# boqian-li/GarmentDreamer

Measured on AMD Instinct MI355X. Metric: SDS iters/sec (rasterize+UNet+bwd), 100k Gaussians ×8 views @512², 1/2/4/8 GPU, higher is better.
Workload: dtype bf16

## Files before the change

garmentdreamer_amd/csrc/nn_conv3x3.hip:

```cpp
#include <hip/hip_runtime.h>
#include <stdlib.h>
#include <stdint.h>
#include <stdio.h>

#include <mutex>
#include <vector>

#include "../../include/gd_nn.h"
#include "nn_device.h"
#include "nn_host.h"

#ifndef GD_CONV_ABLATE
#define GD_CONV_ABLATE 0
#endif

namespace {

using namespace gdnn;

#ifndef GD_PATCH_EPI
#define GD_PATCH_EPI 0
#endif
typedef __attribute__((ext_vector_type(4))) float f32x4;

// ... 241 lines not shown

__device__ __forceinline__ float silu_fast(float z) { return z * __builtin_amdgcn_rcpf(1.0f + __expf(-z)); }

__device__ __forceinline__ float row16_sum(float v)
{
    v += __builtin_bit_cast(float, __builtin_amdgcn_update_dpp(0, __builtin_bit_cast(int, v), 0xB1, 0xf, 0xf, false));
    v += __builtin_bit_cast(float, __builtin_amdgcn_update_dpp(0, __builtin_bit_cast(int, v), 0x4E, 0xf, 0xf, false));
    v += __builtin_bit_cast(float, __builtin_amdgcn_update_dpp(0, __builtin_bit_cast(int, v), 0x141, 0xf, 0xf, false));
    v += __builtin_bit_cast(float, __builtin_amdgcn_update_dpp(0, __builtin_bit_cast(int, v), 0x140, 0xf, 0xf, false));
    return v;
}

__device__ __forceinline__ void stat_accumulate(float2& st, uint2 o)
{
    const float r0 = __uint_as_float(o.x << 16), r1 = __uint_as_float(o.x & 0xffff0000u);
    const float r2 = __uint_as_float(o.y << 16), r3 = __uint_as_float(o.y & 0xffff0000u);
    st.x += (r0 + r1) + (r2 + r3);
    st.y += fmaf(r0, r0, fmaf(r1, r1, fmaf(r2, r2, r3 * r3)));
}

__device__ __forceinline__ void patch_col(int fn, int& rr, int& fx)
{
    if (fn < 4) { rr = 0; fx = fn; }
    else if (fn < 12) { rr = 1; fx = fn - 4; }
    else if (fn < 16) { rr = 0; fx = fn - 8; }
    else if (fn < 20) { rr = 1; fx = fn - 8; }
    else if (fn < 28) { rr = 0; fx = fn - 12; }
    else { rr = 1; fx = fn - 16; }
}

constexpr int kTrRow = 80;
constexpr int kTrWave = 64 * kTrRow;

template <int BN, int WN, int FA, int FB>
__device__ __forceinline__ void patch_epilogue(f32x16 (&acc)[FA][FB], char* tr, int nimg, int tyi, int txi, int n0, int wc,
                                               int wp, int lane, int H, int W, int Cout, const uint16_t* __restrict__ bias,
                                               int bias_img_stride, const uint16_t* __restrict__ residual,
                                               uint16_t* __restrict__ out, float* __restrict__ stat_part, int tpi,
                                               int tiles_x)
{
    const int fk = lane >> 5, fn = lane & 31;
    int rr, fx;
    patch_col(fn, rr, fx);
    bool ok[FB];
    size_t opix[FB];
#pragma unroll
    for (int b = 0; b < FB; b++) {
        const int oy = tyi * 16 + 4 * wp + 2 * b + rr, ox = txi * 16 + fx;
        ok[b] = oy < H && ox < W;
        opix[b] = ((size_t)nimg * H + oy) * W + ox;
    }
    const uint16_t* bias_n = bias ? bias + (size_t)nimg * bias_img_stride : nullptr;
    const int stat_rows = tpi * 8;
    const int stat_row = (tyi * tiles_x + txi) * 8 + wp * 2 + ((lane >> 4) & 1);
    const bool wide = GD_PATCH_EPI != 2 && tr != nullptr && (Cout & 7) == 0;
#pragma unroll
    for (int a = 0; a < FA; a++) {
#pragma unroll
        for (int q = 0; q < 4; q++) {
            const int co = n0 + wc * (BN / WN) + a * 32 + 8 * q + 4 * fk;
            const bool cok = co < Cout;
            float bv[4] = {0.f, 0.f, 0.f, 0.f};
            if (bias_n && cok) {
                const uint2 bb = *(const uint2*)(bias_n + co);
                bv[0] = bf2f((uint16_t)(bb.x & 0xffff)); bv[1] = bf2f((uint16_t)(bb.x >> 16));
                bv[2] = bf2f((uint16_t)(bb.y & 0xffff)); bv[3] = bf2f((uint16_t)(bb.y >> 16));
// ... 13 lines not shown
                uint2 o;
                o.x = pack_bf16(v[0], v[1]);
                o.y = pack_bf16(v[2], v[3]);
                if (wide) *(uint2*)(tr + (b * 32 + fn) * kTrRow + 16 * q + 8 * fk) = o;
                else if (GD_PATCH_EPI != 1 || H < 0) *(uint2*)(out + opix[b] * Cout + co) = o;
                if (stat_part) stat_accumulate(st, o);
            }
            if (stat_part) {
                const float sx = row16_sum(st.x), sy = row16_sum(st.y);
                if ((lane & 15) == 0 && cok)
                    *(float2*)(stat_part + (((size_t)nimg * (Cout >> 2) + (co >> 2)) * stat_rows + stat_row) * 2) =
                        make_float2(sx, sy);
            }
        }
        if (wide) {
            __builtin_amdgcn_wave_barrier();
#pragma unroll
            for (int i = 0; i < FB * 2; i++) {
                const int pr = (lane >> 2) + 16 * i, ch = lane & 3;
                int rr2, fx2;
                patch_col(pr & 31, rr2, fx2);
                const int oy = tyi * 16 + 4 * wp + 2 * (pr >> 5) + rr2, ox = txi * 16 + fx2;
                const int co8 = n0 + wc * (BN / WN) + a * 32 + 8 * ch;
                if (oy < H && ox < W && co8 < Cout) {
                    const uint4 v = *(const uint4*)(tr + pr * kTrRow + ch * 16);
                    if (GD_PATCH_EPI != 1 || H < 0) *(uint4*)(out + (((size_t)nimg * H + oy) * W + ox) * Cout + co8) = v;
                }
            }
            __builtin_amdgcn_wave_barrier();
        }
    }
}

template <int BN, int WN, int WM, bool GN>
__global__ __launch_bounds__(64 * WN * WM) void conv3x3_gn_patch_kernel(
    const uint16_t* __restrict__ in, const uint16_t* __restrict__ wt, const uint16_t* __restrict__ bias,
    int bias_img_stride, const uint16_t* __restrict__ residual, uint16_t* __restrict__ out, int Nimg, int H, int W,
    int Cin, int Cout, const float* __restrict__ mean_rstd, const uint16_t* __restrict__ gamma,
    const uint16_t* __restrict__ beta, int G, int apply_silu, int tiles_n, int tiles_x, int tiles_y, int nwg,
    float* __restrict__ stat_part)
{
    constexpr int BM = 256;
    constexpr int THREADS = 64 * WN * WM;
    constexpr int NB = BN * 8 / THREADS;
    constexpr int NA = (kPatchPix * 8 + THREADS - 1) / THREADS;
    constexpr int FA = BN / WN / 32, FB = BM / WM / 32;
    static_assert(FB == 2 && THREADS % 8 == 0, "wave pixel block = 4 patch rows x 16");
    constexpr int kAStage = (kPatchPix + 4) * BK * 2;
    constexpr int kBStage = BN * BK * 2;
    extern __shared__ __attribute__((aligned(16))) char smem[];
    char* sA = smem;
    char* sB = smem + 2 * kAStage;

    const int tid = threadIdx.x, lane = tid & 63;
    const int wave = __builtin_amdgcn_readfirstlane(tid >> 6);
    int bid = blockIdx.x;
    if ((nwg & 7) == 0) bid = (bid & 7) * (nwg >> 3) + (bid >> 3);
    const int tn = bid % tiles_n, tm = bid / tiles_n;
    const int tpi = tiles_x * tiles_y;
    const int nimg = tm / tpi, trem = tm - nimg * tpi;
    const int tyi = trem / tiles_x, txi = trem - tyi * tiles_x;
    const int y0 = tyi * 16 - 1, x0 = txi * 16 - 1;
    const int n0 = tn * BN;

    const uint32_t row_bytes = (uint32_t)Cin * 2u;
    const __amdgpu_buffer_rsrc_t rs_in = buffer_rsrc(in, (uint32_t)Nimg * (uint32_t)(H * W) * row_bytes);
    const __amdgpu_buffer_rsrc_t rs_w = buffer_rsrc(wt, (uint32_t)Cout * 9u * row_bytes);
// ... 72 lines not shown
#pragma unroll
    for (int a = 0; a < FA; a++)
#pragma unroll
        for (int b = 0; b < FB; b++)
#pragma unroll
            for (int k = 0; k < 16; k++) acc[a][b][k] = 0.f;

    const int wc = wave % WN, wp = wave / WN;
    const int fk = lane >> 5, fn = lane & 31;
    int rr, fx;
    if (fn < 4) { rr = 0; fx = fn; }
    else if (fn < 12) { rr = 1; fx = fn - 4; }
    else if (fn < 16) { rr = 0; fx = fn - 8; }
    else if (fn < 20) { rr = 1; fx = fn - 8; }
    else if (fn < 28) { rr = 0; fx = fn - 12; }
    else { rr = 1; fx = fn - 16; }
    uint32_t w_rd[FA];
    int p_base[FB];
#pragma unroll
    for (int a = 0; a < FA; a++) w_rd[a] = (uint32_t)swz(wc * (BN / WN) + a * 32 + fn, fk);
#pragma unroll
    for (int b = 0; b < FB; b++) p_base[b] = (4 * wp + 2 * b + rr) * kPatch + fx;

    const int kc = Cin / BK;
    const int nsteps = 9 * kc;
    auto issueA = [&](int buf, int c) {
        char* dst = sA + buf * kAStage;
#pragma unroll
        for (int i = 0; i < NA; i++) {
            if (i == NA - 1 && wave * 64 + THREADS * i >= kPatchPix * 8) continue;
            bload_lds16(rs_in, a_goff[i], (uint32_t)c * (BK * 2), dst + (wave * 64 + THREADS * i) * 16);
        }
    };
    if (GN) {
        if (mean_rstd) gn_table_fill(tab_off, tid, THREADS, Cin, G, nimg, mean_rstd, gamma, beta);
        loadA(0);
        issueB(0, 0, 0);
        if (mean_rstd) gn_table_sync();
        storeA(0, 0);
    } else {
        issueA(0, 0);
        issueB(0, 0, 0);
    }
    int s = 0;
    for (int c = 0; c < kc; c++) {
        const char* pa = sA + (c & 1) * kAStage;
        for (int tap = 0; tap < 9; tap++, s++) {
            const int bufB = s & 1;
            if (GN) asm volatile("s_waitcnt vmcnt(0) lgkmcnt(0)" ::: "memory");
            else asm volatile("s_waitcnt vmcnt(0)" ::: "memory");
            __syncthreads();
            if (s + 1 < nsteps) issueB(bufB ^ 1, tap == 8 ? 0 : tap + 1, tap == 8 ? c + 1 : c);
            if (c + 1 < kc) {
                if (GN) {
                    if (tap == 0) loadA(c + 1);
                    else if (tap == 1) storeA((c + 1) & 1, c + 1);
                } else if (tap == 0) {
                    issueA((c + 1) & 1, c + 1);
                }
            }
            const char* pb = sB + bufB * kBStage;
            const int tapoff = (tap / 3) * kPatch + (tap % 3);
            uint32_t p_rd[FB], p_sw[FB];
#pragma unroll
            for (int b = 0; b < FB; b++) {
                const int p = p_base[b] + tapoff;
                p_rd[b] = (uint32_t)p * 128u;
                p_sw[b] = (uint32_t)((p >> 1) & 7);
            }
#pragma unroll
            for (int kk = 0; kk < 4; kk++) {
                bf16x8_t wf[FA], pf[FB];
#pragma unroll
                for (int a = 0; a < FA; a++) wf[a] = *(const bf16x8_t*)(pb + (w_rd[a] ^ (uint32_t)(kk << 5)));
#pragma unroll
                for (int b = 0; b < FB; b++)
                    pf[b] = *(const bf16x8_t*)(pa + p_rd[b] + ((((uint32_t)(2 * kk + fk)) ^ p_sw[b]) << 4));
#pragma unroll
                for (int a = 0; a < FA; a++)
#pragma unroll
                    for (int b = 0; b < FB; b++)
                        acc[a][b] = __builtin_amdgcn_mfma_f32_32x32x16_bf16(wf[a], pf[b], acc[a][b], 0, 0, 0);
            }
        }
    }

    if (GD_PATCH_EPI != 2) __syncthreads();
    patch_epilogue<BN, WN, FA, FB>(acc, sA + ((kc - 1) & 1) * kAStage + wave * kTrWave, nimg, tyi, txi, n0, wc, wp, lane, H, W,
                                   Cout, bias, bias_img_stride, residual, out, stat_part, tpi, tiles_x);
}

template <int BN, int WN, int WM, bool GN>
__global__ __launch_bounds__(64 * WN * WM) void conv3x3_patch_stream_kernel(
    const uint16_t* __restrict__ in, const uint16_t* __restrict__ wt, const uint16_t* __restrict__ bias,
    int bias_img_stride, const uint16_t* __restrict__ residual, uint16_t* __restrict__ out, int Nimg, int H, int W,
    int Cin, int Cout, const float* __restrict__ mean_rstd, const uint16_t* __restrict__ gamma,
    const uint16_t* __restrict__ beta, int G, int apply_silu, int tiles_n, int tiles_x, int tiles_y, int nwg,
    float* __restrict__ stat_part)
{
    constexpr int BM = 256;
    constexpr int THREADS = 64 * WN * WM;
    constexpr int NB = BN * 8 / THREADS;
    constexpr int NA = (kPatchPix * 8 + THREADS - 1) / THREADS;
    constexpr int FA = BN / WN / 32, FB = BM / WM / 32;
    static_assert(FB == 2 && THREADS % 8 == 0, "wave pixel block = 4 patch rows x 16");
    constexpr int kAStage = (kPatchPix + 4) * BK * 2;
    constexpr int kBStage = BN * BK * 2;
    extern __shared__ __attribute__((aligned(16))) char smem[];
    char* sA = smem;
    char* sB = smem + 2 * kAStage;

    const int tid = threadIdx.x, lane = tid & 63;
    const int wave = __builtin_amdgcn_readfirstlane(tid >> 6);
    const int tpi = tiles_x * tiles_y;
    const bool remap = (nwg & 7) == 0 && (GN || (gridDim.x & 7) == 0);
    struct Tile { int nimg, tyi, txi, n0; };
    auto decode = [&](int vb) {
        int bid = vb;
        if (remap) bid = (vb & 7) * (nwg >> 3) + (vb >> 3);
        const int tn = bid % tiles_n, tm = bid / tiles_n;
// ... 764 lines not shown
        hipLaunchKernelGGL(kern, dim3(nmax, 1, ncls), dim3(64 * WN_ * WM_), lds, s, (const uint16_t*)x,            \
                           (const uint16_t*)bias, bias_img_stride, (const uint16_t*)residual, (uint16_t*)y, N, gs, \
                           Cin, Cout, tiles_n);                                                                    \
    } while (0)
    if (variant == 2) GD_LAUNCH_M(256, 256, 2, 4);
    else if (variant == 1) GD_LAUNCH_M(128, 256, 2, 4);
    else GD_LAUNCH_M(128, 128, 2, 2);
#undef GD_LAUNCH_M
    prof.close(flops, bytes);
    const int r = launch_status();
    return r < 0 ? r : 1;
}

static int launch_patch(void* stream, const void* x, const float* mean_rstd, const void* gamma, const void* beta,
                        int groups, int apply_silu, const void* weight, const void* bias, int bias_img_stride,
                        const void* residual, void* y, int N, int H, int W, int Cin, int Cout,
                        float* stat_part = nullptr)
{
    if (!x || !weight || !y) return fail(GD_NN_ERR_INVALID_ARG, "null pointer");
    if (N <= 0 || H <= 0 || W <= 0 || Cin % BK || Cout % 4 || Cin <= 0 || Cout <= 0)
        return fail(GD_NN_ERR_INVALID_ARG, "conv3x3_gn: need Cin % 64 == 0 and Cout % 4 == 0");
    if (mean_rstd && (!gamma || !beta || groups <= 0 || Cin % groups))
        return fail(GD_NN_ERR_INVALID_ARG, "conv3x3_gn: GroupNorm needs gamma, beta and Cin % groups == 0");
    if ((double)N * H * W * Cin * 2.0 >= 2147483648.0 || (double)Cout * 9.0 * Cin * 2.0 >= 2147483648.0)
        return fail(GD_NN_ERR_INVALID_ARG, "conv3x3_gn: activation / weight tensor must be < 2 GiB (32-bit buffer offsets)");
    const TiledArgs a = {stream, x, mean_rstd, gamma, beta, groups, apply_silu, weight, bias, bias_img_stride, residual, y,
                         N, H, W, Cin, Cout, stat_part};
    int bn = (Cout % 256 == 0) ? 256 : 128;
    if (g_force_variant == 1 || g_force_variant == 0) bn = 128;
    if (g_force_variant == 2) bn = 256;
    const bool persistent = conv_env().patch_persistent != 0;
    constexpr auto lds = [](int slab) { return 2 * (kPatchPix + 4) * BK * 2 + 2 * slab * BK * 2; };
    if (mean_rstd && bn == 256 && !gn_table_fits(lds(256), Cin)) bn = 128;
    if (bn == 256)
        return mean_rstd ? launch_tiled<conv3x3_gn_patch_kernel<256, 2, 4, true>>(a, lds(256), 16, 256, false)
                         : launch_tiled<conv3x3_patch_stream_kernel<256, 2, 4, false>>(a, lds(256), 16, 256, persistent);
    return mean_rstd ? launch_tiled<conv3x3_gn_patch_kernel<128, 2, 4, true>>(a, lds(128), 16, 128, false)
                     : launch_tiled<conv3x3_patch_stream_kernel<128, 2, 4, false>>(a, lds(128), 16, 128, persistent);
}


static bool prefer_patch(int N, int H, int W, int Cout)
{
    if (g_force_variant >= 0 || g_force_split >= 0) return g_force_variant == 3;
    if (Cout < 64 || H < 16 || W < 16) return false;
    const int bn = Cout % 256 == 0 ? 256 : 128;
    const int64_t wgs = (int64_t)N * g_route_scale * ((H + 15) / 16) * ((W + 15) / 16) * ((Cout + bn - 1) / bn);
    return wgs >= 256;
}

size_t gd_nn_conv3x3_ws_bytes(int N, int H, int W, int Cin, int Cout)
{
    if (N <= 0 || H <= 0 || W <= 0 || Cout <= 0) return 0;
    if (prefer_patch(N, H, W, Cout)) return 0;
    const int64_t M = (int64_t)N * H * W;
    const int split = choose_split(M, Cout, 9, Cin);
    return split > 1 ? split_ws_bytes(split, M, Cout) : 0;
}

int gd_nn_conv_force_split(int s)
{
    g_force_split = s;
    return GD_NN_OK;
}

int gd_nn_conv_set_route_scale(int k)
{
    if (k < 1) return fail(GD_NN_ERR_INVALID_ARG, "conv route scale must be >= 1");
    g_route_scale = k;
    return GD_NN_OK;
}
// ... 60 lines not shown
    return (size_t)((Cout + 127) / 128) * 3 * (size_t)(Cin / kWinoCK) * (size_t)kWinoWStage;
}

int gd_nn_conv3x3_wino_weights(void* stream, const void* weight, void* u, int Cout, int Cin)
{
    if (!weight || !u || Cout <= 0 || Cin <= 0) return fail(GD_NN_ERR_INVALID_ARG, "wino_weights: bad argument");
    if (Cin % kWinoCK) return fail(GD_NN_ERR_INVALID_ARG, "wino_weights: Cin % 32 != 0");
    const size_t total = gd_nn_conv3x3_wino_weights_bytes(Cout, Cin) / 16;
    const int grid = (int)((total + 255) / 256 < 4096 ? (total + 255) / 256 : 4096);
    hipLaunchKernelGGL(conv3x3_wino_weights_kernel, dim3(grid), dim3(256), 0, (hipStream_t)stream, (const uint16_t*)weight,
                       (uint16_t*)u, Cout, Cin);
    return launch_status();
}

int gd_nn_conv3x3_wino_supported(int N, int H, int W, int Cin, int Cout)
{
    if (N <= 0 || H < 16 || W < 16 || Cin <= 0 || Cout < 64) return 0;
    if (Cin % kWinoCK || Cout % 8) return 0;
    if ((double)N * H * W * Cin * 2.0 >= 2147483648.0 || (double)gd_nn_conv3x3_wino_weights_bytes(Cout, Cin) >= 2147483648.0) return 0;
    return 1;
}

static int launch_wino(void* stream, const void* x, const float* mean_rstd, const void* gamma, const void* beta, int groups,
                       int apply_silu, const void* u, const void* bias, int bias_img_stride, const void* residual, void* y,
                       int N, int H, int W, int Cin, int Cout, float* stat_part)
{
    if (!x || !u || !y) return fail(GD_NN_ERR_INVALID_ARG, "null pointer");
    if (!gd_nn_conv3x3_wino_supported(N, H, W, Cin, Cout))
        return fail(GD_NN_ERR_INVALID_ARG, "conv3x3_wino: need Cin % 32 == 0, Cout % 8 == 0, Cout >= 64, H, W >= 16, tensors < 2 GiB");
    if (mean_rstd && (!gamma || !beta || groups <= 0 || Cin % groups))
        return fail(GD_NN_ERR_INVALID_ARG, "conv3x3_wino: GroupNorm needs gamma, beta and Cin % groups == 0");
    const TiledArgs a = {stream, x, mean_rstd, gamma, beta, groups, apply_silu, u, bias, bias_img_stride, residual, y,
                         N, H, W, Cin, Cout, stat_part};
    return mean_rstd ? launch_tiled<conv3x3_wino_kernel<true>>(a, kWinoLds, 16, 128, false)
                     : launch_tiled<conv3x3_wino_kernel<false>>(a, kWinoLds, 16, 128, false);
}

int gd_nn_conv3x3_wino_forward(void* stream, const void* x, const void* u, const void* bias, int bias_img_stride,
                               const void* residual, void* y, int N, int H, int W, int Cin, int Cout, float* stat_part)
{
    return launch_wino(stream, x, nullptr, nullptr, nullptr, 0, 0, u, bias, bias_img_stride, residual, y, N, H, W, Cin,
                       Cout, stat_part);
}

int gd_nn_conv3x3_wino_gn_forward(void* stream, const void* x, const float* mean_rstd, const void* gamma, const void* beta,
                                  int groups, int apply_silu, const void* u, const void* bias, int bias_img_stride,
                                  const void* residual, void* y, int N, int H, int W, int Cin, int Cout, float* stat_part)
{
    if (!mean_rstd) return fail(GD_NN_ERR_INVALID_ARG, "conv3x3_wino_gn: mean_rstd is NULL");
    return launch_wino(stream, x, mean_rstd, gamma, beta, groups, apply_silu, u, bias, bias_img_stride, residual, y, N, H, W,
                       Cin, Cout, stat_part);
}

size_t gd_nn_conv3x3_wide_weights_bytes(int Cout, int Cin)
{
    if (Cout <= 0 || Cin <= 0 || Cin % kWideCK) return 0;
    return (size_t)((Cout + 127) / 128) * 3 * (size_t)(Cin / kWideCK) * (size_t)kWideWStage;
}

int gd_nn_conv3x3_wide_weights(void* stream, const void* weight, void* u, int Cout, int Cin)
{
    if (!weight || !u || Cout <= 0 || Cin <= 0 || Cin % kWideCK) return fail(GD_NN_ERR_INVALID_ARG, "wide_weights: bad argument");
    const size_t total = gd_nn_conv3x3_wide_weights_bytes(Cout, Cin) / 16;
    const int grid = (int)((total + 255) / 256 < 4096 ? (total + 255) / 256 : 4096);
    hipLaunchKernelGGL(conv3x3_wide_weights_kernel, dim3(grid), dim3(256), 0, (hipStream_t)stream, (const uint16_t*)weight,
                       (uint16_t*)u, Cout, Cin);
    return launch_status();
}

#ifdef GD_NN_EXPERIMENTAL_STREAM
#include "nn_conv_stream_api.h"
#endif

int gd_nn_conv3x3_wide_supported(int N, int H, int W, int Cin, int Cout)
{
    if (N <= 0 || H < 16 || W < 16 || Cin <= 0 || Cout < 64) return 0;
    if (Cin % kWideCK || Cout % 8) return 0;
    if ((double)N * H * W * Cin * 2.0 >= 2147483648.0 || (double)gd_nn_conv3x3_wide_weights_bytes(Cout, Cin) >= 2147483648.0) return 0;
    return 1;
}

static int launch_wide(void* stream, const void* x, const float* mean_rstd, const void* gamma, const void* beta, int groups,
                       int apply_silu, const void* u, const void* bias, int bias_img_stride, const void* residual, void* y,
                       int N, int H, int W, int Cin, int Cout, float* stat_part)
{
    if (!x || !u || !y) return fail(GD_NN_ERR_INVALID_ARG, "null pointer");
    if (!gd_nn_conv3x3_wide_supported(N, H, W, Cin, Cout))
        return fail(GD_NN_ERR_INVALID_ARG, "conv3x3_wide: need Cin % 32 == 0, Cout % 8 == 0, Cout >= 64, H, W >= 16, tensors < 2 GiB");
    if (mean_rstd && (!gamma || !beta || groups <= 0 || Cin % groups))
        return fail(GD_NN_ERR_INVALID_ARG, "conv3x3_wide: GroupNorm needs gamma, beta and Cin % groups == 0");
    const TiledArgs a = {stream, x, mean_rstd, gamma, beta, groups, apply_silu, u, bias, bias_img_stride, residual, y,
                         N, H, W, Cin, Cout, stat_part};
    return mean_rstd ? launch_tiled<conv3x3_wide_kernel<true>>(a, kWideLds, 32, 128, false)
                     : launch_tiled<conv3x3_wide_kernel<false>>(a, kWideLds, 32, 128, false);
}

int gd_nn_conv3x3_wide_forward(void* stream, const void* x, const void* u, const void* bias, int bias_img_stride,
                               const void* residual, void* y, int N, int H, int W, int Cin, int Cout, float* stat_part)
{
    return launch_wide(stream, x, nullptr, nullptr, nullptr, 0, 0, u, bias, bias_img_stride, residual, y, N, H, W, Cin,
                       Cout, stat_part);
}

int gd_nn_conv3x3_wide_gn_forward(void* stream, const void* x, const float* mean_rstd, const void* gamma, const void* beta,
                                  int groups, int apply_silu, const void* u, const void* bias, int bias_img_stride,
                                  const void* residual, void* y, int N, int H, int W, int Cin, int Cout, float* stat_part)
{
    if (!mean_rstd) return fail(GD_NN_ERR_INVALID_ARG, "conv3x3_wide_gn: mean_rstd is NULL");
    return launch_wide(stream, x, mean_rstd, gamma, beta, groups, apply_silu, u, bias, bias_img_stride, residual, y, N, H, W,
                       Cin, Cout, stat_part);
}

#ifdef GD_NN_EXPERIMENTAL_REGW
#include "nn_conv_regw_api.h"
#endif

static int first_mfma_grid(int N, int H, int W)
{
    const int64_t tiles = (int64_t)N * H * ((W + 31) / 32);
    int64_t grid = (tiles + 3) / 4;
    const int64_t cap = 512;
    if (grid > cap) grid = cap;
    return (int)(grid < 1 ? 1 : grid);
}

size_t gd_nn_conv3x3_first_stat_rows(int N, int H, int W, int Cin, int Cout)
{
// ... 291 lines not shown
```

garmentdreamer_amd/csrc/nn_conv_wide.h:

```cpp
#pragma once
#include "nn_device.h"

constexpr int kWideCK = 32;
constexpr int kWidePW = 34, kWidePix = 18 * kWidePW;
constexpr int kWidePStage = 2560 * 16;
constexpr int kWideWStage = 3 * 128 * kWideCK * 2;
constexpr int kWideLds = 2 * kWidePStage + 2 * kWideWStage;

__global__ __launch_bounds__(256) void conv3x3_wide_weights_kernel(const uint16_t* __restrict__ w, uint16_t* __restrict__ u,
                                                                   int Cout, int Cin)
{
    const int kc = Cin / kWideCK;
    const int tiles_n = (Cout + 127) / 128;
    const size_t total = (size_t)tiles_n * 3 * kc * 1536;
    for (size_t i = (size_t)blockIdx.x * blockDim.x + threadIdx.x; i < total; i += (size_t)gridDim.x * blockDim.x) {
        const int q = (int)(i % 1536);
        const size_t sl = i / 1536;
        const int c = (int)(sl % kc);
        const int ky = (int)((sl / kc) % 3);
        const int tn = (int)(sl / kc / 3);
        const int pc = q & 3, row = (q >> 2) & 127, kx = q >> 9;
        const int co = tn * 128 + row;
        const int ci0 = c * kWideCK + ((pc ^ ((row >> 2) & 3)) << 3);
        uint4 v = make_uint4(0u, 0u, 0u, 0u);
        if (co < Cout) v = *(const uint4*)(w + (((size_t)co * 3 + ky) * 3 + kx) * Cin + ci0);
        *(uint4*)(u + i * 8) = v;
    }
}

template <bool GN>
__global__ __launch_bounds__(512) void conv3x3_wide_kernel(
    const uint16_t* __restrict__ in, const uint16_t* __restrict__ uw, const uint16_t* __restrict__ bias,
    int bias_img_stride, const uint16_t* __restrict__ residual, uint16_t* __restrict__ out, int Nimg, int H, int W,
    int Cin, int Cout, const float* __restrict__ mean_rstd, const uint16_t* __restrict__ gamma,
    const uint16_t* __restrict__ beta, int G, int apply_silu, int tiles_n, int tiles_x, int tiles_y, int nwg,
    float* __restrict__ stat_part)
{
    constexpr int THREADS = 512;
    typedef __attribute__((ext_vector_type(4))) uint32_t u32x4;
    extern __shared__ __attribute__((aligned(16))) char smem[];
    char* sP = smem;
    char* sW = smem + 2 * kWidePStage;

    const int tid = threadIdx.x, lane = tid & 63;
    const int wave = __builtin_amdgcn_readfirstlane(tid >> 6);
    int bid = blockIdx.x;
    if ((nwg & 7) == 0) bid = (bid & 7) * (nwg >> 3) + (bid >> 3);
    const int tn = bid % tiles_n, tm = bid / tiles_n;
    const int tpi = tiles_x * tiles_y;
    const int nimg = tm / tpi, trem = tm - nimg * tpi;
    const int tyi = trem / tiles_x, txi = trem - tyi * tiles_x;
    const int y0 = tyi * 16 - 1, x0 = txi * 32 - 1;
    const int n0 = tn * 128;

    const uint32_t row_bytes = (uint32_t)Cin * 2u;
    const __amdgpu_buffer_rsrc_t rs_in = buffer_rsrc(in, (uint32_t)Nimg * (uint32_t)(H * W) * row_bytes);
    const int kc = Cin / kWideCK;
    const __amdgpu_buffer_rsrc_t rs_w = buffer_rsrc(uw, (uint32_t)tiles_n * 3u * (uint32_t)kc * (uint32_t)kWideWStage);

    uint32_t p_goff[5];
    uint32_t p_keep = 0;
#pragma unroll
    for (int i = 0; i < 5; i++) {
        const int q = tid + THREADS * i;
        const int pix = q >> 2;
        const int py = (pix * 1928) >> 16, px = pix - py * kWidePW;
        const int gy = y0 + py, gx = x0 + px;
        const bool inimg = (pix < kWidePix) & ((unsigned)gy < (unsigned)H) & ((unsigned)gx < (unsigned)W);
        const int oct = GN ? (q & 3) : (q & 3) ^ ((pix >> 2) & 3);
        p_goff[i] = inimg ? (uint32_t)((nimg * H + gy) * W + gx) * row_bytes + (uint32_t)oct * 16u : kOOB;
        if (inimg) p_keep |= 1u << i;
    }
    auto issueP = [&](int buf, int c) {
        char* dst = sP + buf * kWidePStage;
#pragma unroll
        for (int i = 0; i < 5; i++) {
            if (i == 4 && wave == 7) continue;
            bload_lds16(rs_in, p_goff[i], (uint32_t)c * (kWideCK * 2), dst + (wave * 64 + THREADS * i) * 16);
        }
    };
    u32x4 p_reg[3];
    auto loadP = [&](int c, int i0, int i1) {
#pragma unroll
        for (int i = i0; i < i1; i++) {
            if (i == 4 && wave == 7) continue;
            p_reg[i - i0] = __builtin_bit_cast(u32x4, __builtin_amdgcn_raw_buffer_load_b128(rs_in, (int)p_goff[i],
                                                                                         (int)(c * (kWideCK * 2)), 0));
        }
    };
    const uint32_t sP_off = (uint32_t)(uintptr_t)sP;
    const uint32_t tab_off = (uint32_t)(uintptr_t)(smem + kWideLds);
    auto storeP = [&](int buf, int c, int i0, int i1) {
        float sc[8], sh[8];
        gn_table_read(tab_off, c * (kWideCK / 8) + (tid & 3), sc, sh);
#pragma unroll
        for (int i = i0; i < i1; i++) {
            if (i == 4 && wave == 7) continue;
            const int q = tid + THREADS * i, pix = q >> 2;
            const bool keep = (p_keep >> i) & 1u;
            u32x4 v;
#pragma unroll
            for (int k = 0; k < 4; k++) {
                float lo = __uint_as_float(p_reg[i - i0][k] << 16), hi = __uint_as_float(p_reg[i - i0][k] & 0xffff0000u);
                lo = lo * sc[2 * k] + sh[2 * k];
                hi = hi * sc[2 * k + 1] + sh[2 * k + 1];
                if (apply_silu) { lo = silu_fast(lo); hi = silu_fast(hi); }
                v[k] = keep ? pack_bf16(lo, hi) : 0u;
            }
            asm volatile("ds_write_b128 %0, %1" ::"v"(sP_off + (uint32_t)(buf * kWidePStage) + (uint32_t)pix * 64u +
                                                       (uint32_t)(((q & 3) ^ ((pix >> 2) & 3)) << 4)), "v"(v) : "memory");
        }
    };
    const uint32_t w_voff = (uint32_t)tid * 16u;
    auto issueW = [&](int buf, int ky, int c) {
        char* dst = sW + buf * kWideWStage;
        const uint32_t soff = (uint32_t)((tn * 3 + ky) * kc + c) * (uint32_t)kWideWStage;
#pragma unroll
        for (int i = 0; i < 3; i++)
            bload_lds16(rs_w, w_voff + (uint32_t)(THREADS * 16 * i), soff, dst + (wave * 64 + THREADS * i) * 16);
    };

    const int wc = wave & 1, wr = wave >> 1;
    const int fk = lane >> 5, fn = lane & 31;
    int rr, fx;
    patch_col(fn, rr, fx);
    f32x16 acc[2][4];
#pragma unroll
    for (int a = 0; a < 2; a++)
#pragma unroll
        for (int b = 0; b < 4; b++)
#pragma unroll
            for (int k = 0; k < 16; k++) acc[a][b][k] = 0.f;
    int p_base[4];
#pragma unroll
    for (int b = 0; b < 4; b++) p_base[b] = (4 * wr + 2 * (b & 1) + rr) * kWidePW + 16 * (b >> 1) + fx;
    uint32_t a_rd[2];
#pragma unroll
    for (int a = 0; a < 2; a++) a_rd[a] = (uint32_t)((wc * 64 + a * 32 + fn) * 64);
    const uint32_t a_key = (uint32_t)((fn >> 2) & 3);

    const int nsteps = 3 * kc;
    if (GN) {
        gn_table_fill(tab_off, tid, THREADS, Cin, G, nimg, mean_rstd, gamma, beta);
        loadP(0, 0, 3);
        gn_table_sync();
        storeP(0, 0, 0, 3); loadP(0, 3, 5); storeP(0, 0, 3, 5);
    } else {
        issueP(0, 0);
    }
    issueW(0, 0, 0);
    int s = 0;
    for (int c = 0; c < kc; c++) {
        const char* pa = sP + (c & 1) * kWidePStage;
        for (int ky = 0; ky < 3; ky++, s++) {
            const int bufW = s & 1;
            asm volatile("s_waitcnt vmcnt(0) lgkmcnt(0)" ::: "memory");
            __syncthreads();
            if (s + 1 < nsteps) issueW(bufW ^ 1, ky == 2 ? 0 : ky + 1, ky == 2 ? c + 1 : c);
            if (c + 1 < kc) {
                if (GN) {
                    if (ky == 0) loadP(c + 1, 0, 3);
                    else if (ky == 1) { storeP((c + 1) & 1, c + 1, 0, 3); loadP(c + 1, 3, 5); }
                    else storeP((c + 1) & 1, c + 1, 3, 5);
                } else if (ky == 0) {
                    issueP((c + 1) & 1, c + 1);
                }
            }
            const char* pw = sW + bufW * kWideWStage;
#pragma unroll 1
            for (int kx = 0; kx < 3; kx++) {
                uint32_t p_rd[4], p_sw[4];
#pragma unroll
                for (int b = 0; b < 4; b++) {
                    const int p = p_base[b] + ky * kWidePW + kx;
                    p_rd[b] = (uint32_t)p * 64u;
                    p_sw[b] = (uint32_t)((p >> 2) & 3);
                }
#pragma unroll
                for (int kk = 0; kk < 2; kk++) {
                    const uint32_t ch = (uint32_t)(kk * 2 + fk);
                    bf16x8_t wf[2], pf[4];
#pragma unroll
                    for (int a = 0; a < 2; a++)
                        wf[a] = *(const bf16x8_t*)(pw + kx * (128 * 64) + a_rd[a] + ((ch ^ a_key) << 4));
#pragma unroll
                    for (int b = 0; b < 4; b++) pf[b] = *(const bf16x8_t*)(pa + p_rd[b] + ((ch ^ p_sw[b]) << 4));
#pragma unroll
                    for (int a = 0; a < 2; a++)
#pragma unroll
                        for (int b = 0; b < 4; b++)
                            acc[a][b] = __builtin_amdgcn_mfma_f32_32x32x16_bf16(wf[a], pf[b], acc[a][b], 0, 0, 0);
                }
            }
        }
    }

    __syncthreads();
    char* tr = smem + wave * kTrWave;
    const uint16_t* bias_n = bias ? bias + (size_t)nimg * bias_img_stride : nullptr;
    const int stat_rows = ((H + 15) / 16) * ((W + 15) / 16) * 8;
#pragma unroll
    for (int bh = 0; bh < 2; bh++) {
        bool ok[2];
        size_t opix[2];
#pragma unroll
        for (int j = 0; j < 2; j++) {
            const int oy = tyi * 16 + 4 * wr + 2 * j + rr, ox = txi * 32 + 16 * bh + fx;
            ok[j] = oy < H && ox < W;
            opix[j] = ((size_t)nimg * H + oy) * W + ox;
        }
        const int t16x = (W + 15) / 16, cx = 2 * txi + bh;
        const int stat_row = (tyi * t16x + cx) * 8 + wr * 2 + ((lane >> 4) & 1);
#pragma unroll
        for (int a = 0; a < 2; a++) {
#pragma unroll
            for (int q = 0; q < 4; q++) {
                const int co = n0 + wc * 64 + a * 32 + 8 * q + 4 * fk;
                const bool cok = co < Cout;
                float bv[4] = {0.f, 0.f, 0.f, 0.f};
                if (bias_n && cok) {
                    const uint2 bb = *(const uint2*)(bias_n + co);
                    bv[0] = bf2f((uint16_t)(bb.x & 0xffff)); bv[1] = bf2f((uint16_t)(bb.x >> 16));
                    bv[2] = bf2f((uint16_t)(bb.y & 0xffff)); bv[3] = bf2f((uint16_t)(bb.y >> 16));
                }
                float2 st = make_float2(0.f, 0.f);
#pragma unroll
                for (int j = 0; j < 2; j++) {
                    if (!ok[j] || !cok) continue;
                    const int b = 2 * bh + j;
                    float v[4];
// ... 38 lines not shown
```

garmentdreamer_amd/csrc/nn_conv_wino.h:

```cpp
#pragma once
#include "nn_device.h"

#ifndef GD_WINO_ABLATE
#define GD_WINO_ABLATE 0
#endif

constexpr int kWinoCK = 32;
constexpr int kWinoVStage = 4 * 18 * 8 * kWinoCK * 2;
constexpr int kWinoWStage = 4 * 128 * kWinoCK * 2;
constexpr int kWinoPBytes = 21 * 1024;
constexpr int kWinoLds = 2 * kWinoVStage + 2 * kWinoWStage + kWinoPBytes;

__device__ __forceinline__ uint16_t f2bf_finite(float f)
{
    uint32_t u = __float_as_uint(f);
    u += 0x7fffu + ((u >> 16) & 1u);
    return (uint16_t)(u >> 16);
}

__global__ __launch_bounds__(256) void conv3x3_wino_weights_kernel(const uint16_t* __restrict__ w,
                                                                   uint16_t* __restrict__ u, int Cout, int Cin)
{
    const int kc = Cin / kWinoCK;
    const int tiles_n = (Cout + 127) / 128;
    const size_t total = (size_t)tiles_n * 3 * kc * 2048;
    for (size_t i = (size_t)blockIdx.x * blockDim.x + threadIdx.x; i < total; i += (size_t)gridDim.x * blockDim.x) {
        const int q = (int)(i & 2047);
        const size_t sl = i >> 11;
        const int c = (int)(sl % kc);
        const int ky = (int)((sl / kc) % 3);
        const int tn = (int)(sl / kc / 3);
        const int pc = q & 3, row = (q >> 2) & 127, pos = q >> 9;
        const int co = tn * 128 + row;
        const int ci0 = c * kWinoCK + ((pc ^ ((row >> 2) & 3)) << 3);
        uint16_t o[8];
#pragma unroll
        for (int e = 0; e < 8; e++) {
            uint16_t v = 0;
            if (co < Cout) {
                const uint16_t* g = w + ((size_t)co * 3 + ky) * 3 * Cin + ci0 + e;
                const float g0 = bf2f(g[0]), g1 = bf2f(g[Cin]), g2 = bf2f(g[2 * Cin]);
                v = pos == 0 ? g[0] : pos == 3 ? g[2 * Cin]
                    : pos == 1 ? f2bf_finite(0.5f * ((g0 + g2) + g1)) : f2bf_finite(0.5f * ((g0 + g2) - g1));
            }
            o[e] = v;
        }
        *(uint4*)(u + i * 8) = *(const uint4*)o;
    }
}

template <bool GN>
__global__ __launch_bounds__(512) void conv3x3_wino_kernel(
    const uint16_t* __restrict__ in, const uint16_t* __restrict__ uw, const uint16_t* __restrict__ bias,
    int bias_img_stride, const uint16_t* __restrict__ residual, uint16_t* __restrict__ out, int Nimg, int H, int W,
    int Cin, int Cout, const float* __restrict__ mean_rstd, const uint16_t* __restrict__ gamma,
    const uint16_t* __restrict__ beta, int G, int apply_silu, int tiles_n, int tiles_x, int tiles_y, int nwg,
    float* __restrict__ stat_part)
{
    constexpr int BN = 128;
    constexpr int THREADS = 512;
    typedef __attribute__((ext_vector_type(4))) uint32_t u32x4;
    extern __shared__ __attribute__((aligned(16))) char smem[];
    char* sV = smem;
    char* sW = smem + 2 * kWinoVStage;
    char* sP = smem + 2 * kWinoVStage + 2 * kWinoWStage;

    const int tid = threadIdx.x, lane = tid & 63;
    const int wave = __builtin_amdgcn_readfirstlane(tid >> 6);
    int bid = blockIdx.x;
    if ((nwg & 7) == 0) bid = (bid & 7) * (nwg >> 3) + (bid >> 3);
    const int tn = bid % tiles_n, tm = bid / tiles_n;
    const int tpi = tiles_x * tiles_y;
    const int nimg = tm / tpi, trem = tm - nimg * tpi;
    const int tyi = trem / tiles_x, txi = trem - tyi * tiles_x;
    const int y0 = tyi * 16 - 1, x0 = txi * 16 - 1;
    const int n0 = tn * BN;

    const uint32_t row_bytes = (uint32_t)Cin * 2u;
    const __amdgpu_buffer_rsrc_t rs_in = buffer_rsrc(in, (uint32_t)Nimg * (uint32_t)(H * W) * row_bytes);
    const int kc = Cin / kWinoCK;
    const __amdgpu_buffer_rsrc_t rs_w = buffer_rsrc(uw, (uint32_t)tiles_n * 3u * (uint32_t)kc * (uint32_t)kWinoWStage);

    uint32_t p_goff[3];
    uint32_t p_keep = 0;
// ... 174 lines not shown
        for (int a = 0; a < 2; a++)
#pragma unroll
            for (int b = 0; b < 2; b++) {
#pragma unroll
                for (int q = 0; q < 4; q++) {
                    f32x4 sd;
#pragma unroll
                    for (int e = 0; e < 4; e++) sd[e] = pp ? acc[0][a][b][4 * q + e] : acc[1][a][b][4 * q + e];
                    *(f32x4*)(mine + ((a * 2 + b) * 4 + q) * 1024 + lane * 16) = sd;
                }
            }
    }
    __syncthreads();
    {
        const char* theirs = smem + (wave ^ 1) * 16384;
#pragma unroll
        for (int a = 0; a < 2; a++)
#pragma unroll
            for (int b = 0; b < 2; b++)
#pragma unroll
                for (int q = 0; q < 4; q++) {
                    const f32x4 rv = GD_WINO_ABLATE == 5 ? f32x4{0.f, 1.f, 2.f, 3.f}
                                                         : *(const f32x4*)(theirs + ((a * 2 + b) * 4 + q) * 1024 + lane * 16);
#pragma unroll
                    for (int e = 0; e < 4; e++) {
                        const float sm = acc[0][a][b][4 * q + e] + acc[1][a][b][4 * q + e];
                        acc[0][a][b][4 * q + e] = pp ? rv[e] - sm : sm + rv[e];
                    }
                }
    }
    __syncthreads();

    char* tr = smem + wave * kTrWave;
    bool ok[2];
    size_t opix[2];
#pragma unroll
    for (int b = 0; b < 2; b++) {
        const int oy = tyi * 16 + wq * 8 + b * 4 + (fn >> 3), ox = txi * 16 + 2 * (fn & 7) + pp;
        ok[b] = oy < H && ox < W;
        opix[b] = ((size_t)nimg * H + oy) * W + ox;
    }
    const uint16_t* bias_n = bias ? bias + (size_t)nimg * bias_img_stride : nullptr;
    const int stat_rows = tpi * 8;
    const int stat_row = (tyi * tiles_x + txi) * 8 + (pp * 2 + wq) * 2 + ((lane >> 4) & 1);
    const bool wide = (Cout & 7) == 0;
#pragma unroll
    for (int a = 0; a < 2; a++) {
#pragma unroll
        for (int q = 0; q < 4; q++) {
            const int co = n0 + wc * 64 + a * 32 + 8 * q + 4 * fk;
            const bool cok = co < Cout;
            float bv[4] = {0.f, 0.f, 0.f, 0.f};
            if (bias_n && cok) {
                const uint2 bb = *(const uint2*)(bias_n + co);
                bv[0] = bf2f((uint16_t)(bb.x & 0xffff)); bv[1] = bf2f((uint16_t)(bb.x >> 16));
                bv[2] = bf2f((uint16_t)(bb.y & 0xffff)); bv[3] = bf2f((uint16_t)(bb.y >> 16));
            }
            float2 st = make_float2(0.f, 0.f);
#pragma unroll
            for (int b = 0; b < 2; b++) {
                if (!ok[b] || !cok) continue;
                float v[4];
#pragma unroll
                for (int e = 0; e < 4; e++) v[e] = acc[0][a][b][4 * q + e] + bv[e];
                if (residual) {
                    const uint2 rv = *(const uint2*)(residual + opix[b] * Cout + co);
// ... 34 lines not shown
```

Baseline: 22.80.

## Prefetch residual tiles into LDS via buffer loads in conv3x3 epilogues

Adds a residual-fused epilogue path for the patch, Winograd and wide conv3x3 kernels. The residual tile is fetched with buffer-to-LDS loads, issued during the last K step and between epilogue rounds, so it overlaps with compute instead of going through per-lane global reads in the epilogue. The new path applies only to full interior tiles with Cout a multiple of 8 and tensors under 4 GiB. It reuses freed operand staging buffers for the residual slots, raises the wide kernel's LDS size when a residual is present, and adds template instantiations.

```diff
diff --git a/garmentdreamer_amd/csrc/nn_conv3x3.hip b/garmentdreamer_amd/csrc/nn_conv3x3.hip
--- a/garmentdreamer_amd/csrc/nn_conv3x3.hip
+++ b/garmentdreamer_amd/csrc/nn_conv3x3.hip
@@ -297,6 +297,115 @@
 constexpr int kTrRow = 80;
 constexpr int kTrWave = 64 * kTrRow;
 
+constexpr int kResRound = 64 * 64;
+
+__device__ __forceinline__ void res_tile_lane(int lane, uint32_t pix_bytes, uint32_t img_row_bytes, uint32_t (&off)[2])
+{
+    const uint32_t chunk = (uint32_t)((lane & 3) ^ ((lane >> 4) & 3));
+#pragma unroll
+    for (int h = 0; h < 2; h++) {
+        int rr, fx;
+        patch_col(16 * h + (lane >> 2), rr, fx);
+        off[h] = (uint32_t)rr * img_row_bytes + (uint32_t)fx * pix_bytes + chunk * 16u;
+    }
+}
+
+__device__ __forceinline__ void res_tile_issue(__amdgpu_buffer_rsrc_t rs, const uint32_t (&off)[2], uint32_t base,
+                                               uint32_t two_rows, char* slot)
+{
+#pragma unroll
+    for (int i = 0; i < 4; i++) bload_lds16(rs, off[i & 1], base + (uint32_t)(i >> 1) * two_rows, slot + i * 1024);
+}
+
+typedef __attribute__((ext_vector_type(2))) uint32_t res_u32x2;
+typedef __attribute__((ext_vector_type(4))) uint32_t res_u32x4;
+
+__device__ __forceinline__ void res_tile_read(uint32_t slot_off, int lane, res_u32x2 (&r)[2][4])
+{
+    const int fn = lane & 31, fk = lane >> 5;
+    const uint32_t a0 = slot_off + (uint32_t)(fn * 64 + 8 * fk), key = (uint32_t)((fn >> 2) & 3);
+    const uint32_t q0 = a0 + (key << 4), q1 = a0 + ((1u ^ key) << 4), q2 = a0 + ((2u ^ key) << 4), q3 = a0 + ((3u ^ key) << 4);
+    asm volatile("ds_read_b64 %0, %8\n\tds_read_b64 %1, %9\n\tds_read_b64 %2, %10\n\tds_read_b64 %3, %11\n\t"
+                 "ds_read_b64 %4, %8 offset:2048\n\tds_read_b64 %5, %9 offset:2048\n\t"
+                 "ds_read_b64 %6, %10 offset:2048\n\tds_read_b64 %7, %11 offset:2048\n\ts_waitcnt lgkmcnt(0)"
+                 : "=&v"(r[0][0]), "=&v"(r[0][1]), "=&v"(r[0][2]), "=&v"(r[0][3]), "=&v"(r[1][0]), "=&v"(r[1][1]),
+                   "=&v"(r[1][2]), "=&v"(r[1][3])
+                 : "v"(q0), "v"(q1), "v"(q2), "v"(q3)
+                 : "memory");
+}
+
+struct ResTile {
+    uint16_t* out;
+    size_t pix0;
+    int Cout;
+    float* stat_img;
+    int stat_rows, stat_row;
+    bool stat_ok;
+};
+
+struct PatchPix {
+    int W;
+    __device__ __forceinline__ int operator()(int pr) const
+    {
+        int rr, fx;
+        patch_col(pr & 31, rr, fx);
+        return (2 * (pr >> 5) + rr) * W + fx;
+    }
+};
+
+template <class PixOf, class AfterRead>
+__device__ __forceinline__ void res_round(const f32x16& acc0, const f32x16& acc1, const uint2 (&bb)[4], uint32_t slot_off,
+                                          uint32_t tr_off, int lane, const ResTile& t, int co0, PixOf pix_of,
+                                          AfterRead after_read)
+{
+    const int fk = lane >> 5, fn = lane & 31;
+    res_u32x2 rv[2][4];
+    res_tile_read(slot_off, lane, rv);
+    after_read();
+#pragma unroll
+    for (int q = 0; q < 4; q++) {
+        const int co = co0 + 8 * q + 4 * fk;
+        const float bv[4] = {bf2f((uint16_t)(bb[q].x & 0xffff)), bf2f((uint16_t)(bb[q].x >> 16)),
+                             bf2f((uint16_t)(bb[q].y & 0xffff)), bf2f((uint16_t)(bb[q].y >> 16))};
+        float2 st = make_float2(0.f, 0.f);
+#pragma unroll
+        for (int j = 0; j < 2; j++) {
+            float v[4];
+#pragma unroll
+            for (int e = 0; e < 4; e++) v[e] = (j ? acc1 : acc0)[4 * q + e] + bv[e];
+            const uint32_t r0 = rv[j][q][0], r1 = rv[j][q][1];
+            v[0] += bf2f((uint16_t)(r0 & 0xffff)); v[1] += bf2f((uint16_t)(r0 >> 16));
+            v[2] += bf2f((uint16_t)(r1 & 0xffff)); v[3] += bf2f((uint16_t)(r1 >> 16));
+            uint2 o;
+            o.x = pack_bf16(v[0], v[1]);
+            o.y = pack_bf16(v[2], v[3]);
+            const res_u32x2 ov = {o.x, o.y};
+            asm volatile("ds_write_b64 %0, %1" ::"v"(tr_off + (uint32_t)((j * 32 + fn) * kTrRow + 16 * q + 8 * fk)), "v"(ov)
+                         : "memory");
+            if (t.stat_img) stat_accumulate(st, o);
+        }
+        if (t.stat_img) {
+            const float sx = row16_sum(st.x), sy = row16_sum(st.y);
+            if ((lane & 15) == 0 && t.stat_ok)
+                *(float2*)(t.stat_img + ((size_t)(co >> 2) * t.stat_rows + t.stat_row + ((lane >> 4) & 1)) * 2) =
+                    make_float2(sx, sy);
+        }
+    }
+    res_u32x4 tv[4];
+    asm volatile("ds_read_b128 %0, %4\n\tds_read_b128 %1, %4 offset:1280\n\tds_read_b128 %2, %4 offset:2560\n\t"
+                 "ds_read_b128 %3, %4 offset:3840\n\ts_waitcnt lgkmcnt(0)"
+                 : "=&v"(tv[0]), "=&v"(tv[1]), "=&v"(tv[2]), "=&v"(tv[3])
+                 : "v"(tr_off + (uint32_t)((lane >> 2) * kTrRow + (lane & 3) * 16))
+                 : "memory");
+    static_assert(16 * kTrRow == 1280, "offsets of the four reads");
+#pragma unroll
+    for (int i = 0; i < 4; i++) {
+        const int pr = (lane >> 2) + 16 * i;
+        *(uint4*)(t.out + (t.pix0 + (size_t)pix_of(pr)) * t.Cout + co0 + 8 * (lane & 3)) =
+            make_uint4(tv[i][0], tv[i][1], tv[i][2], tv[i][3]);
+    }
+}
+
 template <int BN, int WN, int FA, int FB>
 __device__ __forceinline__ void patch_epilogue(f32x16 (&acc)[FA][FB], char* tr, int nimg, int tyi, int txi, int n0, int wc,
                                                int wp, int lane, int H, int W, int Cout, const uint16_t* __restrict__ bias,
@@ -376,7 +485,7 @@
     }
 }
 
-template <int BN, int WN, int WM, bool GN>
+template <int BN, int WN, int WM, bool GN, bool RES>
 __global__ __launch_bounds__(64 * WN * WM) void conv3x3_gn_patch_kernel(
     const uint16_t* __restrict__ in, const uint16_t* __restrict__ wt, const uint16_t* __restrict__ bias,
     int bias_img_stride, const uint16_t* __restrict__ residual, uint16_t* __restrict__ out, int Nimg, int H, int W,
@@ -515,6 +624,23 @@
             bload_lds16(rs_in, a_goff[i], (uint32_t)c * (BK * 2), dst + (wave * 64 + THREADS * i) * 16);
         }
     };
+    static_assert(FA == 2 || FA == 4, "rounds of the residual tile");
+    const bool dma = RES && residual != nullptr && (Cout & 7) == 0 && tyi * 16 + 16 <= H && txi * 16 + 16 <= W && n0 + BN <= Cout &&
+                     (uint64_t)Nimg * (uint64_t)(H * W) * (uint64_t)Cout * 2u < (1ull << 32);
+    const uint32_t res_pix = (uint32_t)Cout * 2u, res_row = (uint32_t)W * res_pix;
+    const __amdgpu_buffer_rsrc_t rs_res = buffer_rsrc(residual, (uint32_t)Nimg * (uint32_t)(H * W) * res_pix);
+    auto res_slot = [&](int r) -> char* {
+        if (r == 0 || r == 3) return sA + (kc & 1) * kAStage + wave * kResRound;
+        return sB + (r - 1) * (8 * kResRound) + wave * kResRound;
+    };
+    auto issueR = [&](int r) {
+        uint32_t off[2];
+        res_tile_lane(lane, res_pix, res_row, off);
+        const uint32_t base = (uint32_t)((nimg * H + tyi * 16 + 4 * wp) * W + txi * 16) * res_pix +
+                              (uint32_t)(n0 + wc * (BN / WN) + r * 32) * 2u;
+        res_tile_issue(rs_res, off, base, 2u * res_row, res_slot(r));
+    };
+
     if (GN) {
         if (mean_rstd) gn_table_fill(tab_off, tid, THREADS, Cin, G, nimg, mean_rstd, gamma, beta);
         loadA(0);
@@ -541,6 +667,8 @@
                 } else if (tap == 0) {
                     issueA((c + 1) & 1, c + 1);
                 }
+            } else if (tap == 0 && dma) {
+                issueR(0);
             }
             const char* pb = sB + bufB * kBStage;
             const int tapoff = (tap / 3) * kPatch + (tap % 3);
@@ -569,6 +697,35 @@
     }
 
     if (GD_PATCH_EPI != 2) __syncthreads();
+    if (GD_PATCH_EPI == 0 && dma) {
+        const uint32_t tr_off = (uint32_t)(uintptr_t)(sA + ((kc - 1) & 1) * kAStage + wave * kTrWave);
+        const uint16_t* bias_d = bias ? bias + (size_t)nimg * bias_img_stride : nullptr;
+        uint2 bb[FA][4];
+#pragma unroll
+        for (int a = 0; a < FA; a++)
+#pragma unroll
+            for (int q = 0; q < 4; q++)
+                bb[a][q] = bias_d ? *(const uint2*)(bias_d + n0 + wc * (BN / WN) + a * 32 + 8 * q + 4 * fk) : make_uint2(0u, 0u);
+        asm volatile("" ::: "memory");
+        issueR(1);
+        if (FA == 4) issueR(2);
+        ResTile t;
+        t.out = out; t.Cout = Cout;
+        t.pix0 = ((size_t)nimg * H + (tyi * 16 + 4 * wp)) * W + txi * 16;
+        t.stat_rows = tpi * 8;
+        t.stat_img = stat_part ? stat_part + (size_t)nimg * (Cout >> 2) * t.stat_rows * 2 : nullptr;
+        t.stat_row = (tyi * tiles_x + txi) * 8 + wp * 2;
+        t.stat_ok = true;
+#pragma unroll
+        for (int r = 0; r < FA; r++) {
+            if (r == FA - 3) asm volatile("s_waitcnt vmcnt(8)" ::: "memory");
+            else if (r == FA - 2 && r > 0) asm volatile("s_waitcnt vmcnt(4)" ::: "memory");
+            else if (r == FA - 1) asm volatile("s_waitcnt vmcnt(0)" ::: "memory");
+            res_round(acc[r][0], acc[r][1], bb[r], (uint32_t)(uintptr_t)res_slot(r), tr_off, lane, t,
+                      n0 + wc * (BN / WN) + r * 32, PatchPix{W}, [&] { if (FA == 4 && r == 0) issueR(3); });
+        }
+        return;
+    }
     patch_epilogue<BN, WN, FA, FB>(acc, sA + ((kc - 1) & 1) * kAStage + wave * kTrWave, nimg, tyi, txi, n0, wc, wp, lane, H, W,
                                    Cout, bias, bias_img_stride, residual, out, stat_part, tpi, tiles_x);
 }
@@ -1399,11 +1556,14 @@
     const bool persistent = conv_env().patch_persistent != 0;
     constexpr auto lds = [](int slab) { return 2 * (kPatchPix + 4) * BK * 2 + 2 * slab * BK * 2; };
     if (mean_rstd && bn == 256 && !gn_table_fits(lds(256), Cin)) bn = 128;
-    if (bn == 256)
-        return mean_rstd ? launch_tiled<conv3x3_gn_patch_kernel<256, 2, 4, true>>(a, lds(256), 16, 256, false)
-                         : launch_tiled<conv3x3_patch_stream_kernel<256, 2, 4, false>>(a, lds(256), 16, 256, persistent);
-    return mean_rstd ? launch_tiled<conv3x3_gn_patch_kernel<128, 2, 4, true>>(a, lds(128), 16, 128, false)
-                     : launch_tiled<conv3x3_patch_stream_kernel<128, 2, 4, false>>(a, lds(128), 16, 128, persistent);
+    if (bn == 256) {
+        if (!mean_rstd) return launch_tiled<conv3x3_patch_stream_kernel<256, 2, 4, false>>(a, lds(256), 16, 256, persistent);
+        return residual ? launch_tiled<conv3x3_gn_patch_kernel<256, 2, 4, true, true>>(a, lds(256), 16, 256, false)
+                        : launch_tiled<conv3x3_gn_patch_kernel<256, 2, 4, true, false>>(a, lds(256), 16, 256, false);
+    }
+    if (!mean_rstd) return launch_tiled<conv3x3_patch_stream_kernel<128, 2, 4, false>>(a, lds(128), 16, 128, persistent);
+    return residual ? launch_tiled<conv3x3_gn_patch_kernel<128, 2, 4, true, true>>(a, lds(128), 16, 128, false)
+                    : launch_tiled<conv3x3_gn_patch_kernel<128, 2, 4, true, false>>(a, lds(128), 16, 128, false);
 }
 
 
@@ -1530,8 +1690,11 @@
         return fail(GD_NN_ERR_INVALID_ARG, "conv3x3_wino: GroupNorm needs gamma, beta and Cin % groups == 0");
     const TiledArgs a = {stream, x, mean_rstd, gamma, beta, groups, apply_silu, u, bias, bias_img_stride, residual, y,
                          N, H, W, Cin, Cout, stat_part};
-    return mean_rstd ? launch_tiled<conv3x3_wino_kernel<true>>(a, kWinoLds, 16, 128, false)
-                     : launch_tiled<conv3x3_wino_kernel<false>>(a, kWinoLds, 16, 128, false);
+    if (residual)
+        return mean_rstd ? launch_tiled<conv3x3_wino_kernel<true, true>>(a, kWinoLds, 16, 128, false)
+                         : launch_tiled<conv3x3_wino_kernel<false, true>>(a, kWinoLds, 16, 128, false);
+    return mean_rstd ? launch_tiled<conv3x3_wino_kernel<true, false>>(a, kWinoLds, 16, 128, false)
+                     : launch_tiled<conv3x3_wino_kernel<false, false>>(a, kWinoLds, 16, 128, false);
 }
 
 int gd_nn_conv3x3_wino_forward(void* stream, const void* x, const void* u, const void* bias, int bias_img_stride,
@@ -1589,8 +1752,11 @@
         return fail(GD_NN_ERR_INVALID_ARG, "conv3x3_wide: GroupNorm needs gamma, beta and Cin % groups == 0");
     const TiledArgs a = {stream, x, mean_rstd, gamma, beta, groups, apply_silu, u, bias, bias_img_stride, residual, y,
                          N, H, W, Cin, Cout, stat_part};
-    return mean_rstd ? launch_tiled<conv3x3_wide_kernel<true>>(a, kWideLds, 32, 128, false)
-                     : launch_tiled<conv3x3_wide_kernel<false>>(a, kWideLds, 32, 128, false);
+    if (residual)
+        return mean_rstd ? launch_tiled<conv3x3_wide_kernel<true, true>>(a, kWideLds, 32, 128, false)
+                         : launch_tiled<conv3x3_wide_kernel<false, true>>(a, kWideLds, 32, 128, false);
+    return mean_rstd ? launch_tiled<conv3x3_wide_kernel<true, false>>(a, kWideStages, 32, 128, false)
+                     : launch_tiled<conv3x3_wide_kernel<false, false>>(a, kWideStages, 32, 128, false);
 }
 
 int gd_nn_conv3x3_wide_forward(void* stream, const void* x, const void* u, const void* bias, int bias_img_stride,
diff --git a/garmentdreamer_amd/csrc/nn_conv_wide.h b/garmentdreamer_amd/csrc/nn_conv_wide.h
--- a/garmentdreamer_amd/csrc/nn_conv_wide.h
+++ b/garmentdreamer_amd/csrc/nn_conv_wide.h
@@ -5,7 +5,9 @@
 constexpr int kWidePW = 34, kWidePix = 18 * kWidePW;
 constexpr int kWidePStage = 2560 * 16;
 constexpr int kWideWStage = 3 * 128 * kWideCK * 2;
-constexpr int kWideLds = 2 * kWidePStage + 2 * kWideWStage;
+constexpr int kWideStages = 2 * kWidePStage + 2 * kWideWStage;
+constexpr int kWideRes = 16384;
+constexpr int kWideLds = kWideStages + kWideRes;
 
 __global__ __launch_bounds__(256) void conv3x3_wide_weights_kernel(const uint16_t* __restrict__ w, uint16_t* __restrict__ u,
                                                                    int Cout, int Cin)
@@ -28,7 +30,7 @@
     }
 }
 
-template <bool GN>
+template <bool GN, bool RES>
 __global__ __launch_bounds__(512) void conv3x3_wide_kernel(
     const uint16_t* __restrict__ in, const uint16_t* __restrict__ uw, const uint16_t* __restrict__ bias,
     int bias_img_stride, const uint16_t* __restrict__ residual, uint16_t* __restrict__ out, int Nimg, int H, int W,
@@ -89,7 +91,7 @@
         }
     };
     const uint32_t sP_off = (uint32_t)(uintptr_t)sP;
-    const uint32_t tab_off = (uint32_t)(uintptr_t)(smem + kWideLds);
+    const uint32_t tab_off = (uint32_t)(uintptr_t)(smem + (RES ? kWideLds : kWideStages));
     auto storeP = [&](int buf, int c, int i0, int i1) {
         float sc[8], sh[8];
         gn_table_read(tab_off, c * (kWideCK / 8) + (tid & 3), sc, sh);
@@ -138,6 +140,22 @@
 #pragma unroll
     for (int a = 0; a < 2; a++) a_rd[a] = (uint32_t)((wc * 64 + a * 32 + fn) * 64);
     const uint32_t a_key = (uint32_t)((fn >> 2) & 3);
+
+    const bool dma = RES && residual != nullptr && tyi * 16 + 16 <= H && txi * 32 + 32 <= W && n0 + 128 <= Cout &&
+                     (uint64_t)Nimg * (uint64_t)(H * W) * (uint64_t)Cout * 2u < (1ull << 32);
+    const uint32_t res_pix = (uint32_t)Cout * 2u, res_row = (uint32_t)W * res_pix;
+    const __amdgpu_buffer_rsrc_t rs_res = buffer_rsrc(residual, (uint32_t)Nimg * (uint32_t)(H * W) * res_pix);
+    auto res_slot = [&](int r) -> char* {
+        if (r == 0 || r == 3) return sP + (kc & 1) * kWidePStage + wave * kResRound;
+        return smem + 2 * kWidePStage + (r - 1) * (8 * kResRound) + wave * kResRound;
+    };
+    auto issueR = [&](int r) {
+        uint32_t off[2];
+        res_tile_lane(lane, res_pix, res_row, off);
+        const uint32_t base = (uint32_t)((nimg * H + tyi * 16 + 4 * wr) * W + txi * 32 + 16 * (r >> 1)) * res_pix +
+                              (uint32_t)(n0 + wc * 64 + (r & 1) * 32) * 2u;
+        res_tile_issue(rs_res, off, base, 2u * res_row, res_slot(r));
+    };
 
     const int nsteps = 3 * kc;
     if (GN) {
@@ -165,6 +183,8 @@
                 } else if (ky == 0) {
                     issueP((c + 1) & 1, c + 1);
                 }
+            } else if (ky == 0 && dma) {
+                issueR(0);
             }
             const char* pw = sW + bufW * kWideWStage;
 #pragma unroll 1
@@ -196,6 +216,38 @@
     }
 
     __syncthreads();
+    if (dma) {
+        const uint32_t tr_off = (uint32_t)(uintptr_t)(sP + ((kc - 1) & 1) * kWidePStage + wave * kTrWave);
+        const uint16_t* bias_d = bias ? bias + (size_t)nimg * bias_img_stride : nullptr;
+        uint2 bb[2][4];
+#pragma unroll
+        for (int a = 0; a < 2; a++)
+#pragma unroll
+            for (int q = 0; q < 4; q++)
+                bb[a][q] = bias_d ? *(const uint2*)(bias_d + n0 + wc * 64 + a * 32 + 8 * q + 4 * fk) : make_uint2(0u, 0u);
+        asm volatile("" ::: "memory");
+        issueR(1);
+        issueR(2);
+        ResTile t;
+        t.out = out; t.Cout = Cout;
+        t.stat_rows = ((H + 15) / 16) * ((W + 15) / 16) * 8;
+        t.stat_img = stat_part ? stat_part + (size_t)nimg * (Cout >> 2) * t.stat_rows * 2 : nullptr;
+        const int t16x = (W + 15) / 16;
+#pragma unroll
+        for (int r = 0; r < 4; r++) {
+            const int bh = r >> 1, a = r & 1;
+            if (r == 1) asm volatile("s_waitcnt vmcnt(8)" ::: "memory");
+            else if (r == 2) asm volatile("s_waitcnt vmcnt(4)" ::: "memory");
+            else if (r == 3) asm volatile("s_waitcnt vmcnt(0)" ::: "memory");
+            const int cx = 2 * txi + bh;
+            t.pix0 = ((size_t)nimg * H + (tyi * 16 + 4 * wr)) * W + (txi * 32 + 16 * bh);
+            t.stat_row = (tyi * t16x + cx) * 8 + wr * 2;
+            t.stat_ok = cx < t16x;
+            res_round(acc[a][2 * bh], acc[a][2 * bh + 1], bb[a], (uint32_t)(uintptr_t)res_slot(r), tr_off, lane, t,
+                      n0 + wc * 64 + a * 32, PatchPix{W}, [&] { if (r == 0) issueR(3); });
+        }
+        return;
+    }
     char* tr = smem + wave * kTrWave;
     const uint16_t* bias_n = bias ? bias + (size_t)nimg * bias_img_stride : nullptr;
     const int stat_rows = ((H + 15) / 16) * ((W + 15) / 16) * 8;
diff --git a/garmentdreamer_amd/csrc/nn_conv_wino.h b/garmentdreamer_amd/csrc/nn_conv_wino.h
--- a/garmentdreamer_amd/csrc/nn_conv_wino.h
+++ b/garmentdreamer_amd/csrc/nn_conv_wino.h
@@ -49,7 +49,7 @@
     }
 }
 
-template <bool GN>
+template <bool GN, bool RES>
 __global__ __launch_bounds__(512) void conv3x3_wino_kernel(
     const uint16_t* __restrict__ in, const uint16_t* __restrict__ uw, const uint16_t* __restrict__ bias,
     int bias_img_stride, const uint16_t* __restrict__ residual, uint16_t* __restrict__ out, int Nimg, int H, int W,
@@ -290,6 +290,43 @@
     __syncthreads();
 
     char* tr = smem + wave * kTrWave;
+    if (RES && residual != nullptr && tyi * 16 + 16 <= H && txi * 16 + 16 <= W && n0 + BN <= Cout && (Cout & 7) == 0 &&
+        (uint64_t)Nimg * (uint64_t)(H * W) * (uint64_t)Cout * 2u < (1ull << 32)) {
+        const uint32_t res_pix = (uint32_t)Cout * 2u, res_row = (uint32_t)W * res_pix;
+        const __amdgpu_buffer_rsrc_t rs_res = buffer_rsrc(residual, (uint32_t)Nimg * (uint32_t)(H * W) * res_pix);
+        const uint16_t* bias_d = bias ? bias + (size_t)nimg * bias_img_stride : nullptr;
+        uint2 bb[2][4];
+#pragma unroll
+        for (int a = 0; a < 2; a++)
+#pragma unroll
+            for (int q = 0; q < 4; q++)
+                bb[a][q] = bias_d ? *(const uint2*)(bias_d + n0 + wc * 64 + a * 32 + 8 * q + 4 * fk) : make_uint2(0u, 0u);
+        asm volatile("" ::: "memory");
+        const uint32_t lane_off = (uint32_t)(lane >> 5) * res_row + (uint32_t)(2 * ((lane >> 2) & 7)) * res_pix +
+                                  (uint32_t)(((lane & 3) ^ ((lane >> 4) & 3)) * 16);
+        const uint32_t base = (uint32_t)((nimg * H + tyi * 16 + wq * 8) * W + txi * 16 + pp) * res_pix + (uint32_t)(n0 + wc * 64) * 2u;
+        char* slot = smem + 8 * kTrWave + wave * (2 * kResRound);
+#pragma unroll
+        for (int a = 0; a < 2; a++)
+#pragma unroll
+            for (int i = 0; i < 4; i++)
+                bload_lds16(rs_res, lane_off, base + (uint32_t)(2 * i) * res_row + (uint32_t)(a * 64), slot + a * kResRound + i * 1024);
+        ResTile t;
+        t.out = out; t.Cout = Cout;
+        t.pix0 = ((size_t)nimg * H + (tyi * 16 + wq * 8)) * W + txi * 16 + pp;
+        t.stat_rows = tpi * 8;
+        t.stat_img = stat_part ? stat_part + (size_t)nimg * (Cout >> 2) * t.stat_rows * 2 : nullptr;
+        t.stat_row = (tyi * tiles_x + txi) * 8 + (pp * 2 + wq) * 2;
+        t.stat_ok = true;
+        const auto pix_of = [W](int pr) { return ((pr >> 5) * 4 + ((pr & 31) >> 3)) * W + 2 * (pr & 7); };
+        asm volatile("s_waitcnt vmcnt(4)" ::: "memory");
+        res_round(acc[0][0][0], acc[0][0][1], bb[0], (uint32_t)(uintptr_t)slot, (uint32_t)(uintptr_t)tr, lane, t, n0 + wc * 64,
+                  pix_of, [] {});
+        asm volatile("s_waitcnt vmcnt(0)" ::: "memory");
+        res_round(acc[0][1][0], acc[0][1][1], bb[1], (uint32_t)(uintptr_t)(slot + kResRound), (uint32_t)(uintptr_t)tr, lane, t,
+                  n0 + wc * 64 + 32, pix_of, [] {});
+        return;
+    }
     bool ok[2];
     size_t opix[2];
 #pragma unroll
```

Result: faster. 23.08, median of 6 (+1.2%).
